# 115dkk/Impulcifer-pip313

Hardware: AMD Instinct MI355X
Metric: impulse responses/sec (sweep deconv+FIR), 7.1×2-ear @48kHz, 1/2/4/8 GPU (higher is better)
Workload: dtype f32

## Files before the change

### impulcifer-pip313_amd/csrc/conv_kernels.hip.h

```cpp
#pragma once
#include "fft_regs.hip.h"

namespace imp {

constexpr int kN2 = 4096;
constexpr int kLogN2 = 12;
constexpr int kRowPad = 272;
#ifndef IMP_AB_PREFETCH
#define IMP_AB_PREFETCH 8
#endif
constexpr int kAbPrefetch = IMP_AB_PREFETCH;

struct Twiddles {
  const cf* __restrict__ full;
  const cf* __restrict__ hi;
  const cf* __restrict__ t1;
  const cf* __restrict__ t2;
  const cf* __restrict__ t4;
};

__device__ __forceinline__ void xcd_work_item(int nchan, int& tile, int& chan) {
  const int xcd = blockIdx.x & 7;
  const int slot = blockIdx.x >> 3;
  const int tl = slot / nchan;
// ... 820 lines not shown
}

struct FirBlockArgs {
  const float4* __restrict__ ab;
  long long ab_chan_stride;
  float* __restrict__ out;
  long long out_stride;
  long long out_start, out_len;
  int kp;
  int valid;
  int blocks;
  int first_block;
  int nchan;
};

constexpr int kFirBlockPoints = 4 * kN2;
constexpr size_t kFirBlockLds = sizeof(cf) * 4 * 16 * kRowPad;

template <class L, class = void> struct LoadHasDeviceLen { static constexpr bool value = false; };
template <class L> struct LoadHasDeviceLen<L, decltype((void)L::kDeviceLen)> { static constexpr bool value = true; };

template <class Load>
__global__ __launch_bounds__(1024, 4) void fir_block_kernel(Load ld, FirBlockArgs a, Twiddles tw) {
  extern __shared__ __attribute__((aligned(16))) char smem_raw[];
  cf* lds = reinterpret_cast<cf*>(smem_raw);
  const int xcd = blockIdx.x & 7, slot = blockIdx.x >> 3;
  const int chan = (slot / a.blocks) * 8 + xcd, blk = a.first_block + slot % a.blocks;
  if (chan >= a.nchan) return;
  long long out_len = a.out_len;
  int filt = chan;
  if constexpr (LoadHasDeviceLen<Load>::value) {
    out_len = ld.out_len(chan);
    filt = ld.filter_of(chan);
    if ((long long)blk * a.valid - a.out_start >= out_len) return;
  }
  const int tid = threadIdx.x;
  const int pairq = __builtin_amdgcn_readfirstlane(tid >> 9);
  const int half = __builtin_amdgcn_readfirstlane((tid >> 8) & 1);
  const int t = tid & 255;
  const int k1 = pairq + 2 * half;
  const int s0 = blk * a.valid - a.kp;
  const __amdgpu_buffer_rsrc_t r_full = make_rsrc(tw.full, 4u * kN2 * 8u);
  const auto row = ld.open(chan);

  cf v[16];
#pragma unroll
  for (int h = 0; h < 2; ++h) {
    cf x[2][4], w[2][3];
#pragma unroll
    for (int c = 0; c < 2; ++c) {
      const int n2 = tid + 1024 * (2 * h + c);
#pragma unroll
      for (int n1 = 0; n1 < 4; ++n1) x[c][n1] = row.pair_at(s0 + 2 * (n1 * kN2 + n2));
#pragma unroll
      for (int k = 1; k < 4; ++k) w[c][k - 1] = bload_cf(r_full, (unsigned)(k * kN2 + n2) * 8u, 0u);
    }
#pragma unroll
    for (int c = 0; c < 2; ++c) {
      const int n2 = tid + 1024 * (2 * h + c);
#pragma unroll
      for (int n1 = 0; n1 < 4; ++n1) x[c][n1] = row.finish(x[c][n1], s0 + 2 * (n1 * kN2 + n2));
      bfly4<-1>(x[c][0], x[c][1], x[c][2], x[c][3]);
      lds[n2] = x[c][0];
#pragma unroll
      for (int k = 1; k < 4; ++k) lds[k * kN2 + n2] = cmul(x[c][k], w[c][k - 1]);
    }
  }
  __syncthreads();
#pragma unroll
  for (int j = 0; j < 16; ++j) v[j] = lds[k1 * kN2 + t + 256 * j];
  __syncthreads();
  const __amdgpu_buffer_rsrc_t r_ab =
      make_rsrc(a.ab + (long long)filt * a.ab_chan_stride + (long long)k1 * kN2, kN2 * sizeof(float4));
  rows_core<0, 4>(v, lds + pairq * (2 * 16 * kRowPad), half, pairq, k1, r_ab, tw, t);

  __syncthreads();
#pragma unroll
  for (int j = 0; j < 16; ++j) lds[k1 * kN2 + t + 256 * j] = v[j];
  __syncthreads();
  const __amdgpu_buffer_rsrc_t r_out = make_rsrc(a.out + (long long)chan * a.out_stride, (unsigned)out_len * 4u);
  const int o0 = blk * a.valid - a.kp - (int)a.out_start;
#pragma unroll
  for (int c = 0; c < 4; ++c) {
    const int n2 = tid + 1024 * c;
    cf w0 = lds[n2], w1 = lds[kN2 + n2], w2 = lds[2 * kN2 + n2], w3 = lds[3 * kN2 + n2];
    w1 = cmulc(w1, bload_cf(r_full, (unsigned)(kN2 + n2) * 8u, 0u));
    w2 = cmulc(w2, bload_cf(r_full, (unsigned)(2 * kN2 + n2) * 8u, 0u));
    w3 = cmulc(w3, bload_cf(r_full, (unsigned)(3 * kN2 + n2) * 8u, 0u));
    bfly4<+1>(w0, w1, w2, w3);
    const cf y[4] = {w0, w1, w2, w3};
#pragma unroll
    for (int n1 = 0; n1 < 4; ++n1) {
      const int pos = 2 * (n1 * kN2 + n2);
      if (pos < a.kp) continue;
      const unsigned off = (unsigned)(o0 + pos) * 4u;
      if (a.out_start & 1) {
        unsigned off_im = off + 4u;
        asm volatile("" : "+v"(off_im));
        __builtin_amdgcn_raw_buffer_store_b32(__float_as_uint(y[n1].x), r_out, off, 0u, 0);
        __builtin_amdgcn_raw_buffer_store_b32(__float_as_uint(y[n1].y), r_out, off_im, 0u, 0);
      } else {
        bstore_cf<kStreamAux>(y[n1], r_out, off, 0u);
      }
    }
  }
}

// ... 2 lines not shown
```

### impulcifer-pip313_amd/csrc/impulse_hip.hip

```cpp
#include <hip/hip_runtime.h>

#include <algorithm>
#include <cmath>
#include <complex>
#include <cstdarg>
#include <cstdio>
#include <cstdlib>
#include <cstring>
#include <map>
#include <mutex>
#include <new>
#include <string>
#include <vector>

#include "internal.h"
#include "conv_kernels.hip.h"
#include "ir_kernels.hip.h"
#include "decay_kernels.hip.h"
#include "slice_kernels.hip.h"

static thread_local std::string g_last_error;

int imp_fail(int code, const char* fmt, ...) {
  char buf[1024];
// ... 436 lines not shown
  int64_t nfft = 0, Nc = 0;
  bool ola = false;
  int64_t ola_lb = 0, ola_mp = 0, ola_blocks = 1, ola_parts = 1;
  int N1 = 0, R2 = 0, F = 16;
  int64_t ws_channels = 0;
  int lanes = 1;
  int64_t group_counter_lane = 0;
  hipStream_t cur_stream = nullptr;
  cf* cur_ws = nullptr;
  TwSet tw;
  float4* ab = nullptr;
  cf* ws = nullptr;
  bool fused = false;
  int f_kp = 0, f_valid = 0;
  int64_t f_first = 0, f_blocks = 0;
  bool paired = false;
  cf* hs = nullptr;
  float* d_in = nullptr;
  float* d_out = nullptr;
  size_t d_in_bytes = 0, d_out_bytes = 0;
  unsigned* tile_max = nullptr;
  int timing = 0;
  int64_t group_counter = 0;
  bool group_timed = false;
  std::vector<hipEvent_t> events;
  int64_t timed = 0;
  double acc_ms[3] = {0, 0, 0};
  int64_t acc_launches = 0;
};

// ... 104 lines not shown
  int rc_attr = ctx_kernel_lds(p->ctx, reinterpret_cast<const void*>(imp::rows_single_kernel), kRowsSingleLds);
  if (rc_attr) return rc_attr;
  imp::RowsPairArgs a;
  a.ws = p->cur_ws;
  a.hs = p->hs;
  a.n1_total = p->N1;
  a.npairs = (int)npairs;
  imp::Twiddles tw{p->tw.full, p->tw.hi, p->ctx->tw_t1, p->ctx->tw_t2, p->ctx->tw_t4};
  dim3 grid((unsigned)(npairs * ((p->N1 + 7) / 8 * 8))), block(256);
  hipLaunchKernelGGL(imp::rows_single_kernel, grid, block, kRowsSingleLds, p->cur_stream, a, tw);
  HIP_TRY(hipGetLastError());
  return IMP_OK;
}

static constexpr int64_t kFusedMaxTaps = 24577;

static int plan_geometry(imp_plan* p, int64_t M, int64_t n_filters, int64_t L, int mode, int64_t ws_channels,
                         bool paired = false, bool allow_fused = true) {
  if (M < 1 || L < 1) return fail(IMP_ERR_INVALID, "M and L must be >= 1 (M=%lld L=%lld)", (long long)M, (long long)L);
  if (n_filters < 1) return fail(IMP_ERR_INVALID, "n_filters must be >= 1");
  if (mode != IMP_MODE_SAME && mode != IMP_MODE_FULL) return fail(IMP_ERR_INVALID, "mode must be IMP_MODE_SAME or IMP_MODE_FULL");
  const int64_t full = L + M - 1;
  const int64_t need = (mode == IMP_MODE_SAME) ? std::max(L + M / 2, M) : full;
  static const struct { int f, r2; bool pair_only; } kShapes[] = {
      {4, 1, false},  {8, 1, false},  {16, 1, false}, {8, 3, false},  {16, 2, false},  {8, 5, false},
      {16, 3, false}, {16, 4, false}, {11, 6, false}, {8, 9, false},  {16, 5, false},  {16, 6, false},
      {16, 8, false}, {11, 12, true}, {16, 9, false}, {16, 10, false}, {16, 12, false}, {16, 16, false}, {16, 18, true},
      {16, 24, true}};
  const int64_t samples_per_row = paired ? imp::kN2 : 2 * imp::kN2;
  if (paired && n_filters != 1) return fail(IMP_ERR_INVALID, "pair mode needs ONE filter shared by both channels of a pair");
// ... 89 lines not shown
  if (e != hipSuccess) return fail(IMP_ERR_ALLOC, "hipMalloc(spectrum): %s", hipGetErrorString(e));
  e = hipMalloc((void**)&p->ws, p->fused ? 256 : plane * (size_t)(p->paired ? p->ws_channels / 2 : p->ws_channels) * sizeof(cf));
  if (e != hipSuccess) return fail(IMP_ERR_ALLOC, "hipMalloc(workspace): %s", hipGetErrorString(e));
  return IMP_OK;
}

static int plan_sync_lanes(imp_plan* p);

extern "C" void imp_plan_destroy(imp_plan* p) {
  if (!p) return;
  IMP_CTX_LOCK(p->ctx);
  (void)hipSetDevice(p->ctx->device);
  (void)plan_sync_lanes(p);
  if (p->ab) (void)hipFree(p->ab);
  if (p->hs) (void)hipFree(p->hs);
  if (p->ws) (void)hipFree(p->ws);
  if (p->d_in) (void)hipFree(p->d_in);
  if (p->d_out) (void)hipFree(p->d_out);
  for (auto ev : p->events) (void)hipEventDestroy(ev);
  delete p;
}

static int plan_create_empty_impl(imp_ctx* ctx, int64_t M, int64_t n_filters, int64_t L, int mode, int64_t ws_channels,
                                  bool paired, imp_plan** out, bool allow_fused = true) {
  if (!ctx || !out) return fail(IMP_ERR_INVALID, "imp_conv_plan_create_empty: null argument");
  IMP_CTX_LOCK(ctx);
  *out = nullptr;
  imp_plan* p = new (std::nothrow) imp_plan();
  if (!p) return fail(IMP_ERR_ALLOC, "out of host memory");
  p->ctx = ctx;
// ... 5 lines not shown
  }
  *out = p;
  return IMP_OK;
}

extern "C" int imp_conv_plan_create_empty(imp_ctx* ctx, int64_t M, int64_t n_filters, int64_t L, int mode,
                                          int64_t ws_channels, imp_plan** out) {
  return plan_create_empty_impl(ctx, M, n_filters, L, mode, ws_channels, false, out);
}

extern "C" int imp_conv_plan_create_empty_paired(imp_ctx* ctx, int64_t M, int64_t L, int mode, int64_t ws_channels,
                                                 imp_plan** out) {
  return plan_create_empty_impl(ctx, M, 1, L, mode, ws_channels, true, out);
}

static int plan_fill_spectrum(imp_plan* p, const double* filter, int64_t filter_ld, bool on_device = false) {
  imp_ctx* ctx = p->ctx;
  const int64_t M = p->M, n_filters = p->n_filters;
  const int64_t ld = n_filters > 1 ? filter_ld : M;
  if (on_device) {
    if (p->paired || p->ola) return fail(IMP_ERR_UNSUPPORTED, "device filters: mono and fused plans without overlap-add");
    return spectrum_alpha_beta_device(ctx, filter, M, n_filters, ld, p->Nc, p->N1, p->ab, true);
  }
  if (p->paired) return spectrum_pair_device(ctx, filter, M, p->Nc, p->N1, p->hs);
  const size_t plane = (size_t)p->N1 * imp::kN2;
  const char* host_env = std::getenv("IMPULSE_HIP_HOST_SPECTRUM");
  if (host_env && host_env[0] == '1' && !p->ola) {
    std::vector<float4> ab(plane);
    std::vector<cd> H;
    for (int64_t f = 0; f < n_filters; ++f) {
      host_rfft(filter + f * ld, M, p->Nc, H);
// ... 5 lines not shown
    }
    return IMP_OK;
  }
  if (!p->ola) return spectrum_alpha_beta_device(ctx, filter, M, n_filters, ld, p->Nc, p->N1, p->ab);
  for (int64_t j = 0; j < p->ola_parts; ++j) {
    const int64_t m0 = j * p->ola_mp, mj = std::min(p->ola_mp, M - m0);
    for (int64_t f = 0; f < n_filters; ++f) {
      int rc = spectrum_alpha_beta_device(ctx, filter + f * ld + m0, mj, 1, mj, p->Nc, p->N1,
                                          p->ab + (size_t)(f * p->ola_parts + j) * plane);
      if (rc) return rc;
    }
  }
  return IMP_OK;
}

static int plan_create_impl(imp_ctx* ctx, const double* filter, int64_t M, int64_t n_filters, int64_t filter_ld, int64_t L,
                            int mode, int64_t ws_channels, bool paired, imp_plan** out, bool allow_fused = true) {
  if (!ctx || !out) return fail(IMP_ERR_INVALID, "imp_conv_plan_create: null argument");
  if (!filter) return fail(IMP_ERR_INVALID, "imp_conv_plan_create: null filter");
  IMP_CTX_LOCK(ctx);
  if (n_filters > 1 && filter_ld < M) return fail(IMP_ERR_INVALID, "filter_ld < M");
  imp_plan* p = nullptr;
  int rc = plan_create_empty_impl(ctx, M, n_filters, L, mode, ws_channels, paired, &p, allow_fused);
  if (rc) return rc;
  if ((rc = plan_fill_spectrum(p, filter, filter_ld))) {
    imp_plan_destroy(p);
    return rc;
  }
  *out = p;
  return IMP_OK;
// ... 100 lines not shown
}

extern "C" int imp_plan_info(const imp_plan* p, int64_t* nfft, int64_t* out_len, int64_t* ws_channels,
                             int64_t* n1_rows) {
  if (!p) return fail(IMP_ERR_INVALID, "null plan");
  if (nfft) *nfft = p->nfft;
  if (out_len) *out_len = p->out_len;
  if (ws_channels) *ws_channels = p->ws_channels;
  if (n1_rows) *n1_rows = p->N1;
  return IMP_OK;
}

extern "C" int imp_plan_spectrum(imp_plan* p, void** dptr, size_t* bytes) {
  if (!p || !dptr || !bytes) return fail(IMP_ERR_INVALID, "imp_plan_spectrum: null argument");
  IMP_CTX_LOCK(p->ctx);
  if (p->paired) {
    *dptr = p->hs;
    *bytes = (size_t)p->N1 * imp::kN2 * sizeof(cf);
    return IMP_OK;
  }
  *dptr = p->ab;
  *bytes = (size_t)p->N1 * imp::kN2 * (size_t)(p->n_filters * p->ola_parts) * sizeof(float4);
  return IMP_OK;
}

extern "C" int imp_plan_copy_spectrum(imp_plan* dst, imp_plan* src) {
  if (!dst || !src) return fail(IMP_ERR_INVALID, "imp_plan_copy_spectrum: null argument");
  if (dst == src) return IMP_OK;
  if (dst->paired != src->paired || dst->fused != src->fused || dst->N1 != src->N1 || dst->M != src->M || dst->L != src->L ||
      dst->mode != src->mode || dst->n_filters != src->n_filters || dst->ola_parts != src->ola_parts)
    return fail(IMP_ERR_INVALID, "imp_plan_copy_spectrum: the two plans differ in geometry");
  void *d = nullptr, *s_ = nullptr;
  size_t nd = 0, ns = 0;
  int rc;
  if ((rc = imp_plan_spectrum(src, &s_, &ns)) || (rc = imp_plan_spectrum(dst, &d, &nd))) return rc;
  if (nd != ns) return fail(IMP_ERR_INVALID, "imp_plan_copy_spectrum: spectrum sizes differ");
  {
    IMP_CTX_LOCK(src->ctx);
    if ((rc = ctx_bind(src->ctx))) return rc;
    HIP_TRY(hipStreamSynchronize(src->ctx->stream));
  }
  IMP_CTX_LOCK(dst->ctx);
  if ((rc = ctx_bind(dst->ctx))) return rc;
  if ((rc = plan_sync_lanes(dst))) return rc;
  HIP_TRY(hipMemcpyPeerAsync(d, dst->ctx->device, s_, src->ctx->device, ns, dst->ctx->stream));
  HIP_TRY(hipStreamSynchronize(dst->ctx->stream));
  return IMP_OK;
}

extern "C" int imp_memcpy_peer(imp_ctx* dst_ctx, void* dst, imp_ctx* src_ctx, const void* src, size_t bytes) {
// ... 70 lines not shown
  const size_t need = (size_t)(4 * (p->timed + 1));
  while (p->events.size() < need) {
    hipEvent_t ev;
    HIP_TRY(hipEventCreate(&ev));
    p->events.push_back(ev);
  }
  HIP_TRY(hipEventRecord(p->events[(size_t)(4 * p->timed + slot)], p->cur_stream));
  if (slot == 3) ++p->timed;
  return IMP_OK;
}

template <class Load>
static int run_group_with(imp_plan* p, Load ld, int64_t nchan, float* d_y, int64_t chan_stride_out,
                          int64_t first_chan, int last_stage);

template <class Load>
static int launch_fir_block(imp_plan* p, Load ld, int64_t nchan, float* d_y, int64_t chan_stride_out, int64_t first_chan) {
  auto kern = imp::fir_block_kernel<Load>;
  int rc = ctx_kernel_lds(p->ctx, reinterpret_cast<const void*>(kern), imp::kFirBlockLds);
  if (rc) return rc;
  const int64_t plane = (int64_t)4 * imp::kN2;
  imp::FirBlockArgs a;
  a.ab = p->ab + (p->n_filters > 1 ? first_chan * plane : 0);
  a.ab_chan_stride = p->n_filters > 1 ? plane : 0;
  a.out = d_y;
  a.out_stride = chan_stride_out;
  a.out_start = p->out_start;
  a.first_block = (int)p->f_first;
  a.out_len = p->out_len;
  a.kp = p->f_kp;
  a.valid = p->f_valid;
  a.blocks = (int)p->f_blocks;
  a.nchan = (int)nchan;
  imp::Twiddles tw{p->tw.full, p->tw.hi, p->ctx->tw_t1, p->ctx->tw_t2, p->ctx->tw_t4};
  dim3 grid((unsigned)((nchan + 7) / 8 * 8 * p->f_blocks)), block(1024);
  hipLaunchKernelGGL(kern, grid, block, imp::kFirBlockLds, p->cur_stream, ld, a, tw);
  HIP_TRY(hipGetLastError());
  return IMP_OK;
}

template <class Load>
static int run_group_pair(imp_plan* p, Load ld, int64_t nchan, float* d_y, int64_t chan_stride_out, int last_stage) {
  int rc;
  const int64_t lane_channels = p->ws_channels / p->lanes;
  const int lane = (p->lanes > 1) ? (int)(p->group_counter_lane++ % p->lanes) : 0;
  p->cur_stream = lane ? p->ctx->side_streams[(size_t)(lane - 1)] : p->ctx->stream;
  p->cur_ws = p->ws + (int64_t)lane * (lane_channels / 2) * p->N1 * imp::kN2;
  if (nchan < 1 || nchan > lane_channels || (lane_channels & 1))
    return fail(IMP_ERR_INVALID, "launch group of %lld channels exceeds the workspace lane (%lld, whole pairs)",
                (long long)nchan, (long long)lane_channels);
  const int64_t npairs = (nchan + 1) / 2;
  if ((double)(chan_stride_out + p->out_len) * 4.0 >= 4294967296.0)
    return fail(IMP_ERR_INVALID, "chan_stride_out %lld: a pair's two output rows must lie within 4 GiB", (long long)chan_stride_out);
// ... 388 lines not shown
  int64_t B = 0, n = 0, head = 0, fade_in = 0, fade_out = 0, pitch_ir = 0;
  double peak_height = 0.12589;
  int lanes = 1;
  int sets = 1;
  int64_t calls = 0;
  int tiles = 0;
  int64_t chunks = 0;
  std::vector<float*> d_ir;
  std::vector<unsigned*> d_tile;
  std::vector<imp::RowPeak*> d_res;
  std::vector<hipEvent_t> k1_done;
  std::vector<hipEvent_t> ir_free;
  std::vector<char> ir_busy;
  int64_t* d_meta = nullptr;
  double* d_win = nullptr;
};

struct ChainLock {
  std::unique_lock<std::recursive_mutex> a, b;
  ChainLock(imp_ctx* x, imp_ctx* y) {
    if (x == y) {
      a = std::unique_lock<std::recursive_mutex>(x->mu);
    } else {
      imp_ctx* lo = x < y ? x : y;
      imp_ctx* hi = x < y ? y : x;
      a = std::unique_lock<std::recursive_mutex>(lo->mu);
      b = std::unique_lock<std::recursive_mutex>(hi->mu);
    }
  }
};

extern "C" void imp_chain_destroy(imp_chain* c) {
  if (!c) return;
  ChainLock lk(c->ctx, c->tail_ctx);
  (void)hipSetDevice(c->ctx->device);
  (void)plan_sync_lanes(c->deconv);
  (void)hipStreamSynchronize(c->tail_ctx->stream);
  for (auto p : c->d_ir) (void)hipFree(p);
  for (auto p : c->d_tile) (void)hipFree(p);
  for (auto p : c->d_res) (void)hipFree(p);
  for (auto e : c->k1_done) (void)hipEventDestroy(e);
  for (auto e : c->ir_free) (void)hipEventDestroy(e);
  (void)hipFree(c->d_meta);
  (void)hipFree(c->d_win);
  delete c;
}

extern "C" int imp_chain_create(imp_plan* deconv, imp_plan* fir, int64_t B, int64_t head, int64_t fade_in, int64_t fade_out,
                                double peak_height, imp_chain** out) {
  if (!deconv || !fir || !out) return fail(IMP_ERR_INVALID, "imp_chain_create: null argument");
  *out = nullptr;
  if (deconv->ctx->device != fir->ctx->device) return fail(IMP_ERR_INVALID, "imp_chain_create: the two plans live on different devices");
  ChainLock lk(deconv->ctx, fir->ctx);
  if (deconv->mode != IMP_MODE_SAME || fir->mode != IMP_MODE_FULL)
    return fail(IMP_ERR_INVALID, "imp_chain_create: needs a 'same' deconvolution plan and a 'full' FIR plan");
  if (!(peak_height > 0.0)) return fail(IMP_ERR_INVALID, "imp_chain_create: peak_height must be positive (got %g)", peak_height);
  if (fir->lanes != 1) return fail(IMP_ERR_INVALID, "imp_chain_create: the FIR plan must run in stream order (lanes = 1)");
  if (deconv->lanes > 1 && deconv->ctx == fir->ctx)
    return fail(IMP_ERR_INVALID, "imp_chain_create: a deconvolution plan with several lanes needs the FIR plan on a context of its own "
// ... 48 lines not shown
    unsigned* tile = nullptr;
    imp::RowPeak* res = nullptr;
    hipEvent_t e1 = nullptr, e2 = nullptr;
    ok = hipMalloc((void**)&ir, (size_t)(B * c->pitch_ir) * sizeof(float)) == hipSuccess;
    if (ir) c->d_ir.push_back(ir);
    ok = ok && hipMalloc((void**)&tile, chunk_bytes * (size_t)c->tiles) == hipSuccess;
    if (tile) c->d_tile.push_back(tile);
    ok = ok && hipMalloc((void**)&res, (size_t)B * sizeof(imp::RowPeak)) == hipSuccess;
    if (res) c->d_res.push_back(res);
    ok = ok && hipEventCreateWithFlags(&e1, hipEventDisableTiming) == hipSuccess;
    if (e1) c->k1_done.push_back(e1);
    ok = ok && hipEventCreateWithFlags(&e2, hipEventDisableTiming) == hipSuccess;
    if (e2) c->ir_free.push_back(e2);
  }
  c->ir_busy.assign((size_t)c->sets, 0);
  if (!ok) {
    (void)hipGetLastError();
    imp_chain_destroy(c);
    return fail(IMP_ERR_ALLOC, "imp_chain_create: device allocation failed");
  }
  *out = c;
  return IMP_OK;
}

extern "C" int imp_chain_execute_device(imp_chain* c, const float* d_x, int64_t chan_stride_in, int64_t elem_stride_in,
                                        float* d_out, int64_t chan_stride_out, long long* d_peaks_out) {
  if (!c || !d_x || !d_out) return fail(IMP_ERR_INVALID, "imp_chain_execute_device: null argument");
  ChainLock lk(c->ctx, c->tail_ctx);
  if (chan_stride_out < c->fir->out_len)
    return fail(IMP_ERR_INVALID, "chan_stride_out %lld < out_len %lld", (long long)chan_stride_out, (long long)c->fir->out_len);
// ... 9 lines not shown
  c->deconv->tile_max = c->d_tile[(size_t)l];
  rc = imp_conv_execute_device(c->deconv, d_x, c->B, chan_stride_in, elem_stride_in, c->d_ir[(size_t)l], c->pitch_ir);
  c->deconv->tile_max = nullptr;
  if (rc) return rc;
  if (c->deconv->cur_stream != lane_stream) return fail(IMP_ERR_HIP, "imp_chain_execute_device: lane bookkeeping out of step");
  if (tail != lane_stream) {
    HIP_TRY(hipEventRecord(c->k1_done[(size_t)l], lane_stream));
    HIP_TRY(hipStreamWaitEvent(tail, c->k1_done[(size_t)l], 0));
  }
  hipLaunchKernelGGL(imp::row_first_peak_chunked_kernel, dim3((unsigned)c->B), dim3(imp::kPeakThreads), 0, tail, c->d_ir[(size_t)l],
                     c->d_meta, c->d_meta + c->B, c->deconv->out_start, (const unsigned*)c->d_tile[(size_t)l], c->tiles,
                     (const unsigned*)nullptr, c->chunks, c->d_res[(size_t)l], c->peak_height, d_peaks_out);
  HIP_TRY(hipGetLastError());
  imp::LoadCropAtPeak ld{c->d_ir[(size_t)l], c->pitch_ir, c->deconv->out_len, c->d_res[(size_t)l], c->n, c->head, c->fade_in, c->fade_out,
                         c->d_win};
  if ((rc = run_group_with(c->fir, ld, c->B, d_out, chan_stride_out, 0, 2))) return rc;
  if (tail != lane_stream) {
    HIP_TRY(hipEventRecord(c->ir_free[(size_t)l], tail));
    c->ir_busy[(size_t)l] = 1;
  }
  return IMP_OK;
}

struct imp_segset {
  imp_ctx* ctx = nullptr;
  int64_t B = 0;
  double* e = nullptr;
  int64_t* off = nullptr;
  int64_t* len = nullptr;
  std::vector<int64_t> h_len;
  void* qbuf = nullptr;
  size_t qcap = 0;
  void* keep_a = nullptr;
  void* keep_b = nullptr;
  std::vector<int64_t> keep_host;
// ... 671 lines not shown
```

### impulcifer-pip313_amd/impulse_hip/_native.py

```python
import atexit
import ctypes as C
import os
import threading
import weakref

import numpy as np

_HERE = os.path.dirname(os.path.abspath(__file__))
_DEFAULT_LIB = os.path.normpath(os.path.join(_HERE, "..", "csrc", "libimpulse_hip.so"))

IMP_MODE_SAME = 0
IMP_MODE_FULL = 1
IMP_ERR_UNSUPPORTED = -3


class NativeUnavailable(RuntimeError):
    """libimpulse_hip.so is missing or no MI355X (gfx950) device is usable."""


class NativeError(RuntimeError):

    def __init__(self, code, message):
        super().__init__(f"impulse_hip error {code}: {message}")
        self.code = code
# ... 75 lines not shown
    "imp_plan_kind": (C.c_int, [_vp, C.POINTER(C.c_int)]),
    "imp_conv_execute_device_pairs": (C.c_int, [_vp, _vp, C.c_int, _i64, _i64, _i64, _i64, _vp, _i64]),
    "imp_plan_destroy": (None, [_vp]),
    "imp_plan_info": (C.c_int, [_vp, _pi64, _pi64, _pi64, _pi64]),
    "imp_plan_spectrum": (C.c_int, [_vp, C.POINTER(_vp), C.POINTER(C.c_size_t)]),
    "imp_plan_copy_spectrum": (C.c_int, [_vp, _vp]),
    "imp_memcpy_peer": (C.c_int, [_vp, _vp, _vp, _vp, C.c_size_t]),
    "imp_conv_execute": (C.c_int, [_vp, _pf, _i64, _i64, _pf, _i64]),
    "imp_conv_execute_interleaved": (C.c_int, [_vp, _pf, _i64, _pf, _i64]),
    "imp_conv_execute_device": (C.c_int, [_vp, _vp, _i64, _i64, _i64, _vp, _i64]),
    "imp_conv_execute_device_pcm": (C.c_int, [_vp, _vp, C.c_int, _i64, _i64, _i64, _vp, _i64]),
    "imp_plan_set_overlap": (C.c_int, [_vp, C.c_int]),
    "imp_chain_create": (C.c_int, [_vp, _vp, _i64, _i64, _i64, _i64, C.c_double, C.POINTER(_vp)]),
    "imp_chain_execute_device": (C.c_int, [_vp, _vp, _i64, _i64, _vp, _i64, _vp]),
    "imp_chain_destroy": (None, [_vp]),
    "imp_slice_create": (C.c_int, [_vp, C.POINTER(SliceGeometry), _i64, C.POINTER(_vp)]),
    "imp_slice_destroy": (None, [_vp]),
    "imp_slice_info": (C.c_int, [_vp, _pi64, _pi64, _pi64, _pi64]),
    "imp_slice_set_firs": (C.c_int, [_vp, _pd, _i64]),
    "imp_slice_execute_device": (C.c_int, [_vp, _vp, _i64, _i64, _vp, _i64]),
    "imp_slice_results": (C.c_int, [_vp, C.POINTER(SliceRowResult), C.POINTER(SliceResult)]),
    "imp_slice_set_decay": (C.c_int, [_vp, _pd]),
    "imp_slice_set_alignment": (C.c_int, [_vp, _i64, C.POINTER(C.c_int32), C.POINTER(C.c_int32), C.POINTER(C.c_int32), C.c_int32, _i64]),
    "imp_xcorr_argmax_device": (C.c_int, [_vp, _vp, _pi64, _pi64, _pi64, _pi64, _i64, _pi64, _pd]),
    "imp_shift_rows_device": (C.c_int, [_vp, _vp, _pi64, _pi64, _pi64, _i64, _vp, _pi64]),
    "imp_slice_pack_f64": (C.c_int, [_vp, _vp, _i64, _i64, _vp, _i64]),
    "imp_host_alloc": (C.c_int, [_vp, C.c_size_t, C.POINTER(_vp)]),
    "imp_host_free": (C.c_int, [_vp]),
    "imp_comm_unique_id": (C.c_int, [C.POINTER(C.c_ubyte)]),
    "imp_comm_create": (C.c_int, [_vp, C.POINTER(C.c_ubyte), C.c_int, C.c_int, C.POINTER(_vp)]),
    "imp_comm_destroy": (None, [_vp]),
    "imp_comm_probe": (C.c_int, []),
    "imp_comm_nranks": (C.c_int, [_vp, C.POINTER(C.c_int)]),
    "imp_comm_broadcast": (C.c_int, [_vp, _vp, C.c_size_t, C.c_int]),
    "imp_plan_broadcast_spectrum": (C.c_int, [_vp, _vp, C.c_int, C.POINTER(C.c_size_t)]),
    "imp_plan_set_filters": (C.c_int, [_vp, _pd, _i64]),
    "imp_plan_set_filters_device": (C.c_int, [_vp, _vp, _i64]),
    "imp_curves_equalization_fir_device": (C.c_int, [_vp, _pd, _i64, C.c_int, C.c_double, C.c_double, C.c_double, C.c_double,
                                                     C.c_double, C.c_int, C.c_double, C.c_double, C.c_int, _pd, C.POINTER(_vp), _pi64]),
    "imp_slice_set_firs_device": (C.c_int, [_vp, _vp, _i64]),
    "imp_plan_set_timing": (C.c_int, [_vp, C.c_int]),
    "imp_plan_get_timing": (C.c_int, [_vp, _pd, _pi64, C.c_int]),
    "imp_debug_plan_geometry": (C.c_int, [_i64, _i64, C.c_int, _pi64, _pi64, _pi64]),
    "imp_debug_plan_geometry_fused": (C.c_int, [_i64, _i64, C.c_int, _pi64, _pi64, _pi64, _pi64]),
    "imp_debug_plan_geometry_paired": (C.c_int, [_i64, _i64, C.c_int, _pi64, _pi64, _pi64, _pi64]),
    "imp_debug_host_spectrum": (C.c_int, [_pd, _i64, C.c_int, _pf]),
    "imp_plan_debug_run_stage": (C.c_int, [_vp, _pf, _i64, _i64, C.c_int, _pf]),
    "imp_segset_create": (C.c_int, [_vp, _pd, _pi64, _pi64, _i64, C.POINTER(_vp), _pd]),
    "imp_segset_range_means": (C.c_int, [_vp, _pi64, _pi64, _pi64, _i64, _pd]),
    "imp_segset_destroy": (None, [_vp]),
    "imp_decay_times": (C.c_int, [_vp, _pd, _pi64, _pi64, _i64, _pi64, _pi64, _pd, _pi64, C.c_double, _pd]),
    "imp_decay_times_device": (C.c_int, [_vp, _vp, _pi64, _pi64, _i64, _pi64, _pi64, _pd, _pi64, C.c_double, _pd]),
    "imp_sosfilt": (C.c_int, [_vp, _pd, _i64, _pd, _pi64, _pi64, _i64, _pd]),
    "imp_xcorr_argmax": (C.c_int, [_vp, _pd, _pi64, _pi64, _pd, _pi64, _pi64, _i64, _pi64, _pd]),
    "imp_minphase_fir": (C.c_int, [_vp, _pd, _i64, _i64, C.c_double, _pd]),
    "imp_curves_create": (C.c_int, [_vp, _pd, _i64, C.POINTER(_vp)]),
    "imp_curves_destroy": (None, [_vp]),
    "imp_curves_window_size": (C.c_int, [_vp, C.c_double, C.POINTER(C.c_int)]),
    "imp_curves_smooth": (C.c_int, [_vp, _pd, _i64, C.c_double, C.c_double, C.c_double, C.c_double, _pd]),
# ... 453 lines not shown
        self.ctx = deconv_plan.ctx
        self._lib = self.ctx._lib
        self._plans = (deconv_plan, fir_plan)
        h = _vp()
        _check(self._lib.imp_chain_create(deconv_plan.handle, fir_plan.handle, int(B), int(head), int(fade_in),
                                          int(fade_out), float(peak_height), C.byref(h)))
        self._h = h
        self.ctx._plans.add(self)
        fir_plan.ctx._plans.add(self)

    def execute_device(self, d_x, chan_stride_in, d_out, chan_stride_out, d_peaks=0, elem_stride_in=1):
        if not getattr(self, "_h", None):
            raise NativeError(-1, "the chain is closed (one of its contexts was closed)")
        _check(self._lib.imp_chain_execute_device(self._h, _vp(int(d_x)), int(chan_stride_in), int(elem_stride_in),
                                                  _vp(int(d_out)), int(chan_stride_out), _vp(int(d_peaks)) if d_peaks else None))

    def close(self):
        if getattr(self, "_h", None):
            if all(getattr(p.ctx, "_h", None) for p in self._plans):
                self._lib.imp_chain_destroy(self._h)
            self._h = None

    def __del__(self):
        try:
            self.close()
        except Exception:
            pass


class Slice:
# ... 557 lines not shown
                                       C.byref(a), C.byref(b), C.byref(c)))
    return a.value, b.value, c.value


def plan_geometry_fused(M, L, mode="same"):
    lib = load_library()
    a, b, c, d = _i64(), _i64(), _i64(), _i64()
    rc = lib.imp_debug_plan_geometry_fused(int(M), int(L), {"same": IMP_MODE_SAME, "full": IMP_MODE_FULL}[mode],
                                           C.byref(a), C.byref(b), C.byref(c), C.byref(d))
    if rc == IMP_ERR_UNSUPPORTED:
        return None
    _check(rc)
    return a.value, b.value, c.value, d.value


def plan_geometry_paired(M, L, mode="same"):
    lib = load_library()
    a, b, c, d = _i64(), _i64(), _i64(), _i64()
    rc = lib.imp_debug_plan_geometry_paired(int(M), int(L), {"same": IMP_MODE_SAME, "full": IMP_MODE_FULL}[mode],
                                            C.byref(a), C.byref(b), C.byref(c), C.byref(d))
    if rc == IMP_ERR_UNSUPPORTED:
        return None
    _check(rc)
    return a.value, b.value, c.value, d.value


def host_spectrum(filt, n1_rows):
    lib = load_library()
    f = np.ascontiguousarray(filt, dtype=np.float64)
    out = np.empty((int(n1_rows), 4096, 4), dtype=np.float32)
# ... 77 lines not shown
```

### include/impulse_hip.h

```cpp
#ifndef IMPULSE_HIP_H_
#define IMPULSE_HIP_H_

#include <stdint.h>
#include <stddef.h>

#ifdef __cplusplus
extern "C" {
#endif

#define IMP_OK 0
#define IMP_ERR_INVALID (-1)
#define IMP_ERR_HIP (-2)
#define IMP_ERR_UNSUPPORTED (-3)
#define IMP_ERR_NO_DEVICE (-4)
#define IMP_ERR_ALLOC (-5)

#define IMP_MODE_SAME 0
#define IMP_MODE_FULL 1

typedef struct imp_ctx imp_ctx;
typedef struct imp_plan imp_plan;

const char* imp_version(void);
const char* imp_last_error(void);
// ... 150 lines not shown
                           int64_t* window_out, int32_t* flags_out);
int imp_rows_to_pcm_device(imp_ctx* ctx, const float* d_rows, const int64_t* off, const int64_t* len, int64_t n_rows,
                           const int64_t* row_of_track, int64_t n_tracks, int64_t n_frames, int bits, void* pcm_out);
int imp_magnitude_db_sum_device(imp_ctx* ctx, const float* d_rows, const int64_t* off, const int64_t* len,
                                const int64_t* group, int64_t n_rows, int64_t n_groups, int64_t n, double* db_out);
int imp_magnitude_db_sum_peak_device(imp_ctx* ctx, const float* d_rows, const int64_t* off, const int64_t* len,
                                     const int64_t* group, int64_t n_rows, int64_t n_groups, int64_t n,
                                     double* peak_db_out);

typedef struct imp_chain imp_chain;
int imp_chain_create(imp_plan* deconv, imp_plan* fir, int64_t B, int64_t head, int64_t fade_in, int64_t fade_out,
                     double peak_height, imp_chain** out);
int imp_chain_execute_device(imp_chain* chain, const float* d_x, int64_t chan_stride_in, int64_t elem_stride_in,
                             float* d_out, int64_t chan_stride_out, long long* d_peaks_out);
void imp_chain_destroy(imp_chain* chain);

#define IMP_SLICE_KNEE_GUARD 1
#define IMP_SLICE_KNEE_RANGE 2
#define IMP_SLICE_KEEP_CAP 4
#define IMP_SLICE_FADE 8
#define IMP_SLICE_GAIN_GUARD 16
#define IMP_SLICE_GAIN_NONFINITE 32
#define IMP_SLICE_SHORT 64
#define IMP_SLICE_ALIGN_GUARD 256
#define IMP_SLICE_DECAY_GUARD 128
typedef struct imp_slice imp_slice;
typedef struct imp_slice_geometry {
  int64_t n_pairs;
  int64_t elem_stride;
  int bits;
// ... 66 lines not shown
```

Baseline: 300,700.

## Add 2-row fused FIR block kernel for chain tail with short filters

Templates the fused FIR block kernel on the number of rows (2 or 4). The chain's FIR stage uses a 512-thread, 8192-point block variant when the filter has at most 12289 taps. The tail needs a separate alpha/beta spectrum at the smaller size, so the plan now keeps device copies of the filter taps, uses generation counters to track staleness, and rebuilds the spectrum lazily. The smaller FFT is meant to cut wasted transform work on short filters, at the cost of more blocks and an extra spectrum buffer per chain.

```diff
diff --git a/impulcifer-pip313_amd/csrc/conv_kernels.hip.h b/impulcifer-pip313_amd/csrc/conv_kernels.hip.h
--- a/impulcifer-pip313_amd/csrc/conv_kernels.hip.h
+++ b/impulcifer-pip313_amd/csrc/conv_kernels.hip.h
@@ -858,14 +858,29 @@
   int nchan;
 };
 
-constexpr int kFirBlockPoints = 4 * kN2;
-constexpr size_t kFirBlockLds = sizeof(cf) * 4 * 16 * kRowPad;
+template <int N1>
+struct FirBlockCfg {
+  static_assert(N1 == 2 || N1 == 4, "fir_block_kernel holds two or four rows");
+  static constexpr int kThreads = 256 * N1;
+  static constexpr int kPoints = N1 * kN2;
+  static constexpr size_t kLds = sizeof(cf) * N1 * 16 * kRowPad;
+  static constexpr int kAbPrefetch = N1 == 4 ? 4 : ::imp::kAbPrefetch;
+};
+constexpr int kFirBlockPoints = FirBlockCfg<4>::kPoints;
+constexpr size_t kFirBlockLds = FirBlockCfg<4>::kLds;
 
 template <class L, class = void> struct LoadHasDeviceLen { static constexpr bool value = false; };
 template <class L> struct LoadHasDeviceLen<L, decltype((void)L::kDeviceLen)> { static constexpr bool value = true; };
 
-template <class Load>
-__global__ __launch_bounds__(1024, 4) void fir_block_kernel(Load ld, FirBlockArgs a, Twiddles tw) {
+template <int N1>
+__device__ __forceinline__ cf fir_twiddle(__amdgpu_buffer_rsrc_t r_full, int k1, int n2) {
+  return bload_cf(r_full, (unsigned)((k1 * (4 / N1)) * kN2 + n2) * 8u, 0u);
+}
+
+template <int N1, class Load>
+__global__ __launch_bounds__(FirBlockCfg<N1>::kThreads, 4) void fir_block_kernel(Load ld, FirBlockArgs a, Twiddles tw) {
+  using Cfg = FirBlockCfg<N1>;
+  constexpr int T = Cfg::kThreads;
   extern __shared__ __attribute__((aligned(16))) char smem_raw[];
   cf* lds = reinterpret_cast<cf*>(smem_raw);
   const int xcd = blockIdx.x & 7, slot = blockIdx.x >> 3;
@@ -879,35 +894,38 @@
     if ((long long)blk * a.valid - a.out_start >= out_len) return;
   }
   const int tid = threadIdx.x;
-  const int pairq = __builtin_amdgcn_readfirstlane(tid >> 9);
+  const int pairq = N1 == 4 ? __builtin_amdgcn_readfirstlane(tid >> 9) : 0;
   const int half = __builtin_amdgcn_readfirstlane((tid >> 8) & 1);
   const int t = tid & 255;
-  const int k1 = pairq + 2 * half;
+  const int k1 = pairq + (N1 / 2) * half;
   const int s0 = blk * a.valid - a.kp;
   const __amdgpu_buffer_rsrc_t r_full = make_rsrc(tw.full, 4u * kN2 * 8u);
   const auto row = ld.open(chan);
 
+  constexpr int CPT = kN2 / T;
+  constexpr int CH = 8 / N1;
   cf v[16];
 #pragma unroll
-  for (int h = 0; h < 2; ++h) {
-    cf x[2][4], w[2][3];
-#pragma unroll
-    for (int c = 0; c < 2; ++c) {
-      const int n2 = tid + 1024 * (2 * h + c);
-#pragma unroll
-      for (int n1 = 0; n1 < 4; ++n1) x[c][n1] = row.pair_at(s0 + 2 * (n1 * kN2 + n2));
-#pragma unroll
-      for (int k = 1; k < 4; ++k) w[c][k - 1] = bload_cf(r_full, (unsigned)(k * kN2 + n2) * 8u, 0u);
-    }
-#pragma unroll
-    for (int c = 0; c < 2; ++c) {
-      const int n2 = tid + 1024 * (2 * h + c);
-#pragma unroll
-      for (int n1 = 0; n1 < 4; ++n1) x[c][n1] = row.finish(x[c][n1], s0 + 2 * (n1 * kN2 + n2));
-      bfly4<-1>(x[c][0], x[c][1], x[c][2], x[c][3]);
+  for (int h = 0; h < CPT / CH; ++h) {
+    cf x[CH][N1], w[CH][N1 - 1];
+#pragma unroll
+    for (int c = 0; c < CH; ++c) {
+      const int n2 = tid + T * (CH * h + c);
+#pragma unroll
+      for (int n1 = 0; n1 < N1; ++n1) x[c][n1] = row.pair_at(s0 + 2 * (n1 * kN2 + n2));
+#pragma unroll
+      for (int k = 1; k < N1; ++k) w[c][k - 1] = fir_twiddle<N1>(r_full, k, n2);
+    }
+#pragma unroll
+    for (int c = 0; c < CH; ++c) {
+      const int n2 = tid + T * (CH * h + c);
+#pragma unroll
+      for (int n1 = 0; n1 < N1; ++n1) x[c][n1] = row.finish(x[c][n1], s0 + 2 * (n1 * kN2 + n2));
+      if constexpr (N1 == 4) bfly4<-1>(x[c][0], x[c][1], x[c][2], x[c][3]);
+      else bfly2<-1>(x[c][0], x[c][1]);
       lds[n2] = x[c][0];
 #pragma unroll
-      for (int k = 1; k < 4; ++k) lds[k * kN2 + n2] = cmul(x[c][k], w[c][k - 1]);
+      for (int k = 1; k < N1; ++k) lds[k * kN2 + n2] = cmul(x[c][k], w[c][k - 1]);
     }
   }
   __syncthreads();
@@ -916,7 +934,7 @@
   __syncthreads();
   const __amdgpu_buffer_rsrc_t r_ab =
       make_rsrc(a.ab + (long long)filt * a.ab_chan_stride + (long long)k1 * kN2, kN2 * sizeof(float4));
-  rows_core<0, 4>(v, lds + pairq * (2 * 16 * kRowPad), half, pairq, k1, r_ab, tw, t);
+  rows_core<0, Cfg::kAbPrefetch>(v, lds + pairq * (2 * 16 * kRowPad), half, pairq, k1, r_ab, tw, t);
 
   __syncthreads();
 #pragma unroll
@@ -925,16 +943,17 @@
   const __amdgpu_buffer_rsrc_t r_out = make_rsrc(a.out + (long long)chan * a.out_stride, (unsigned)out_len * 4u);
   const int o0 = blk * a.valid - a.kp - (int)a.out_start;
 #pragma unroll
-  for (int c = 0; c < 4; ++c) {
-    const int n2 = tid + 1024 * c;
-    cf w0 = lds[n2], w1 = lds[kN2 + n2], w2 = lds[2 * kN2 + n2], w3 = lds[3 * kN2 + n2];
-    w1 = cmulc(w1, bload_cf(r_full, (unsigned)(kN2 + n2) * 8u, 0u));
-    w2 = cmulc(w2, bload_cf(r_full, (unsigned)(2 * kN2 + n2) * 8u, 0u));
-    w3 = cmulc(w3, bload_cf(r_full, (unsigned)(3 * kN2 + n2) * 8u, 0u));
-    bfly4<+1>(w0, w1, w2, w3);
-    const cf y[4] = {w0, w1, w2, w3};
-#pragma unroll
-    for (int n1 = 0; n1 < 4; ++n1) {
+  for (int c = 0; c < CPT; ++c) {
+    const int n2 = tid + T * c;
+    cf y[N1];
+#pragma unroll
+    for (int k = 0; k < N1; ++k) y[k] = lds[k * kN2 + n2];
+#pragma unroll
+    for (int k = 1; k < N1; ++k) y[k] = cmulc(y[k], fir_twiddle<N1>(r_full, k, n2));
+    if constexpr (N1 == 4) bfly4<+1>(y[0], y[1], y[2], y[3]);
+    else bfly2<+1>(y[0], y[1]);
+#pragma unroll
+    for (int n1 = 0; n1 < N1; ++n1) {
       const int pos = 2 * (n1 * kN2 + n2);
       if (pos < a.kp) continue;
       const unsigned off = (unsigned)(o0 + pos) * 4u;
diff --git a/impulcifer-pip313_amd/csrc/impulse_hip.hip b/impulcifer-pip313_amd/csrc/impulse_hip.hip
--- a/impulcifer-pip313_amd/csrc/impulse_hip.hip
+++ b/impulcifer-pip313_amd/csrc/impulse_hip.hip
@@ -474,6 +474,8 @@
   bool fused = false;
   int f_kp = 0, f_valid = 0;
   int64_t f_first = 0, f_blocks = 0;
+  int64_t filter_gen = 0, taps_gen = -1;
+  double* d_taps = nullptr;
   bool paired = false;
   cf* hs = nullptr;
   float* d_in = nullptr;
@@ -608,6 +610,7 @@
 }
 
 static constexpr int64_t kFusedMaxTaps = 24577;
+static constexpr int64_t kChainTail2MaxTaps = 16384 - 4096 + 1;
 
 static int plan_geometry(imp_plan* p, int64_t M, int64_t n_filters, int64_t L, int mode, int64_t ws_channels,
                          bool paired = false, bool allow_fused = true) {
@@ -727,6 +730,7 @@
   (void)plan_sync_lanes(p);
   if (p->ab) (void)hipFree(p->ab);
   if (p->hs) (void)hipFree(p->hs);
+  if (p->d_taps) (void)hipFree(p->d_taps);
   if (p->ws) (void)hipFree(p->ws);
   if (p->d_in) (void)hipFree(p->d_in);
   if (p->d_out) (void)hipFree(p->d_out);
@@ -762,7 +766,7 @@
   return plan_create_empty_impl(ctx, M, 1, L, mode, ws_channels, true, out);
 }
 
-static int plan_fill_spectrum(imp_plan* p, const double* filter, int64_t filter_ld, bool on_device = false) {
+static int plan_fill_planes(imp_plan* p, const double* filter, int64_t filter_ld, bool on_device) {
   imp_ctx* ctx = p->ctx;
   const int64_t M = p->M, n_filters = p->n_filters;
   const int64_t ld = n_filters > 1 ? filter_ld : M;
@@ -798,6 +802,24 @@
   return IMP_OK;
 }
 
+static int plan_fill_spectrum(imp_plan* p, const double* filter, int64_t filter_ld, bool on_device = false) {
+  ++p->filter_gen;
+  int rc = plan_fill_planes(p, filter, filter_ld, on_device);
+  if (rc || !p->fused || p->M > kChainTail2MaxTaps) return rc;
+  const int64_t ld = p->n_filters > 1 ? filter_ld : p->M;
+  const size_t row = (size_t)p->M * sizeof(double);
+  if (!p->d_taps && hipMalloc((void**)&p->d_taps, row * (size_t)p->n_filters) != hipSuccess) {
+    (void)hipGetLastError();
+    p->d_taps = nullptr;
+    return IMP_OK;
+  }
+  HIP_TRY(hipMemcpy2DAsync(p->d_taps, row, filter, (size_t)ld * sizeof(double), row, (size_t)p->n_filters,
+                           on_device ? hipMemcpyDeviceToDevice : hipMemcpyHostToDevice, p->ctx->stream));
+  if (!on_device) HIP_TRY(hipStreamSynchronize(p->ctx->stream));
+  p->taps_gen = p->filter_gen;
+  return IMP_OK;
+}
+
 static int plan_create_impl(imp_ctx* ctx, const double* filter, int64_t M, int64_t n_filters, int64_t filter_ld, int64_t L,
                             int mode, int64_t ws_channels, bool paired, imp_plan** out, bool allow_fused = true) {
   if (!ctx || !out) return fail(IMP_ERR_INVALID, "imp_conv_plan_create: null argument");
@@ -928,6 +950,7 @@
 extern "C" int imp_plan_spectrum(imp_plan* p, void** dptr, size_t* bytes) {
   if (!p || !dptr || !bytes) return fail(IMP_ERR_INVALID, "imp_plan_spectrum: null argument");
   IMP_CTX_LOCK(p->ctx);
+  ++p->filter_gen;
   if (p->paired) {
     *dptr = p->hs;
     *bytes = (size_t)p->N1 * imp::kN2 * sizeof(cf);
@@ -947,7 +970,9 @@
   void *d = nullptr, *s_ = nullptr;
   size_t nd = 0, ns = 0;
   int rc;
+  const int64_t src_gen = src->filter_gen;
   if ((rc = imp_plan_spectrum(src, &s_, &ns)) || (rc = imp_plan_spectrum(dst, &d, &nd))) return rc;
+  src->filter_gen = src_gen;
   if (nd != ns) return fail(IMP_ERR_INVALID, "imp_plan_copy_spectrum: spectrum sizes differ");
   {
     IMP_CTX_LOCK(src->ctx);
@@ -1048,29 +1073,36 @@
 static int run_group_with(imp_plan* p, Load ld, int64_t nchan, float* d_y, int64_t chan_stride_out,
                           int64_t first_chan, int last_stage);
 
-template <class Load>
-static int launch_fir_block(imp_plan* p, Load ld, int64_t nchan, float* d_y, int64_t chan_stride_out, int64_t first_chan) {
-  auto kern = imp::fir_block_kernel<Load>;
-  int rc = ctx_kernel_lds(p->ctx, reinterpret_cast<const void*>(kern), imp::kFirBlockLds);
-  if (rc) return rc;
-  const int64_t plane = (int64_t)4 * imp::kN2;
+template <int N1, class Load>
+static int launch_fir_block_rows(imp_plan* p, Load ld, int64_t nchan, float* d_y, int64_t chan_stride_out, const float4* ab,
+                                 int kp, int valid, int64_t first, int64_t blocks) {
+  using Cfg = imp::FirBlockCfg<N1>;
+  auto kern = imp::fir_block_kernel<N1, Load>;
+  int rc = ctx_kernel_lds(p->ctx, reinterpret_cast<const void*>(kern), Cfg::kLds);
+  if (rc) return rc;
   imp::FirBlockArgs a;
-  a.ab = p->ab + (p->n_filters > 1 ? first_chan * plane : 0);
-  a.ab_chan_stride = p->n_filters > 1 ? plane : 0;
+  a.ab = ab;
+  a.ab_chan_stride = p->n_filters > 1 ? (int64_t)N1 * imp::kN2 : 0;
   a.out = d_y;
   a.out_stride = chan_stride_out;
   a.out_start = p->out_start;
-  a.first_block = (int)p->f_first;
+  a.first_block = (int)first;
   a.out_len = p->out_len;
-  a.kp = p->f_kp;
-  a.valid = p->f_valid;
-  a.blocks = (int)p->f_blocks;
+  a.kp = kp;
+  a.valid = valid;
+  a.blocks = (int)blocks;
   a.nchan = (int)nchan;
   imp::Twiddles tw{p->tw.full, p->tw.hi, p->ctx->tw_t1, p->ctx->tw_t2, p->ctx->tw_t4};
-  dim3 grid((unsigned)((nchan + 7) / 8 * 8 * p->f_blocks)), block(1024);
-  hipLaunchKernelGGL(kern, grid, block, imp::kFirBlockLds, p->cur_stream, ld, a, tw);
+  dim3 grid((unsigned)((nchan + 7) / 8 * 8 * blocks)), block(Cfg::kThreads);
+  hipLaunchKernelGGL(kern, grid, block, Cfg::kLds, p->cur_stream, ld, a, tw);
   HIP_TRY(hipGetLastError());
   return IMP_OK;
+}
+
+template <class Load>
+static int launch_fir_block(imp_plan* p, Load ld, int64_t nchan, float* d_y, int64_t chan_stride_out, int64_t first_chan) {
+  const float4* ab = p->ab + (p->n_filters > 1 ? first_chan * (int64_t)imp::kFirBlockPoints : 0);
+  return launch_fir_block_rows<4>(p, ld, nchan, d_y, chan_stride_out, ab, p->f_kp, p->f_valid, p->f_first, p->f_blocks);
 }
 
 template <class Load>
@@ -1489,7 +1521,37 @@
   std::vector<char> ir_busy;
   int64_t* d_meta = nullptr;
   double* d_win = nullptr;
+  float4* d_ab2 = nullptr;
+  int64_t ab2_gen = -1;
+  int t2_kp = 0, t2_valid = 0;
+  int64_t t2_first = 0, t2_blocks = 0;
 };
+
+static bool chain_tail2_geometry(int64_t M, int64_t out_start, int64_t out_len, int* kp, int* valid, int64_t* first,
+                                 int64_t* blocks) {
+  if (M < 1 || M > kChainTail2MaxTaps) return false;
+  *kp = (int)((M - 1 + 1) & ~(int64_t)1);
+  *valid = (int)(2 * imp::FirBlockCfg<2>::kPoints - *kp);
+  *first = out_start / *valid;
+  *blocks = (out_start + out_len - 1) / *valid - *first + 1;
+  return true;
+}
+
+static int chain_tail2_prepare(imp_chain* c, bool* ready) {
+  imp_plan* f = c->fir;
+  *ready = false;
+  if (!c->d_ab2) return IMP_OK;
+  if (c->ab2_gen == f->filter_gen) {
+    *ready = true;
+    return IMP_OK;
+  }
+  if (!f->d_taps || f->taps_gen != f->filter_gen) return IMP_OK;
+  int rc = spectrum_alpha_beta_device(f->ctx, f->d_taps, f->M, f->n_filters, f->M, imp::FirBlockCfg<2>::kPoints, 2, c->d_ab2, true);
+  if (rc) return rc;
+  c->ab2_gen = f->filter_gen;
+  *ready = true;
+  return IMP_OK;
+}
 
 struct ChainLock {
   std::unique_lock<std::recursive_mutex> a, b;
@@ -1518,6 +1580,7 @@
   for (auto e : c->ir_free) (void)hipEventDestroy(e);
   (void)hipFree(c->d_meta);
   (void)hipFree(c->d_win);
+  (void)hipFree(c->d_ab2);
   delete c;
 }
 
@@ -1596,6 +1659,17 @@
     if (e2) c->ir_free.push_back(e2);
   }
   c->ir_busy.assign((size_t)c->sets, 0);
+  const char* k5_env = std::getenv("IMPULSE_HIP_CHAIN_K5");
+  const bool block4 = k5_env && std::strcmp(k5_env, "block4") == 0;
+  if (ok && fir->fused && !block4 &&
+      chain_tail2_geometry(fir->M, fir->out_start, fir->out_len, &c->t2_kp, &c->t2_valid, &c->t2_first, &c->t2_blocks)) {
+    ok = hipMalloc((void**)&c->d_ab2, (size_t)fir->n_filters * imp::FirBlockCfg<2>::kPoints * sizeof(float4)) == hipSuccess;
+    bool ready = false;
+    if (ok && (rc = chain_tail2_prepare(c, &ready))) {
+      imp_chain_destroy(c);
+      return rc;
+    }
+  }
   if (!ok) {
     (void)hipGetLastError();
     imp_chain_destroy(c);
@@ -1635,11 +1709,45 @@
   HIP_TRY(hipGetLastError());
   imp::LoadCropAtPeak ld{c->d_ir[(size_t)l], c->pitch_ir, c->deconv->out_len, c->d_res[(size_t)l], c->n, c->head, c->fade_in, c->fade_out,
                          c->d_win};
-  if ((rc = run_group_with(c->fir, ld, c->B, d_out, chan_stride_out, 0, 2))) return rc;
+  bool tail2 = false;
+  if ((rc = chain_tail2_prepare(c, &tail2))) return rc;
+  if (tail2) {
+    imp_plan* f = c->fir;
+    f->cur_stream = f->ctx->stream;
+    if ((rc = timing_event(f, 0))) return rc;
+    if ((rc = launch_fir_block_rows<2>(f, ld, c->B, d_out, chan_stride_out, c->d_ab2, c->t2_kp, c->t2_valid, c->t2_first,
+                                       c->t2_blocks)))
+      return rc;
+    for (int slot = 1; slot <= 3; ++slot)
+      if ((rc = timing_event(f, slot))) return rc;
+  } else if ((rc = run_group_with(c->fir, ld, c->B, d_out, chan_stride_out, 0, 2))) {
+    return rc;
+  }
   if (tail != lane_stream) {
     HIP_TRY(hipEventRecord(c->ir_free[(size_t)l], tail));
     c->ir_busy[(size_t)l] = 1;
   }
+  return IMP_OK;
+}
+
+extern "C" int imp_chain_tail_rows(imp_chain* c, int* rows) {
+  if (!c || !rows) return fail(IMP_ERR_INVALID, "imp_chain_tail_rows: null argument");
+  ChainLock lk(c->ctx, c->tail_ctx);
+  imp_plan* f = c->fir;
+  *rows = c->d_ab2 && (c->ab2_gen == f->filter_gen || (f->d_taps && f->taps_gen == f->filter_gen)) ? 2 : 4;
+  return IMP_OK;
+}
+
+extern "C" int imp_debug_chain_tail_geometry(int64_t M, int64_t L, int64_t* history, int64_t* valid, int64_t* blocks) {
+  if (L < 1) return fail(IMP_ERR_INVALID, "L must be >= 1 (got %lld)", (long long)L);
+  int kp = 0, v = 0;
+  int64_t first = 0, nb = 0;
+  if (!chain_tail2_geometry(M, 0, L + M - 1, &kp, &v, &first, &nb))
+    return fail(IMP_ERR_UNSUPPORTED, "the chain's 2-row K5 takes 1 to %lld taps (got %lld)", (long long)kChainTail2MaxTaps,
+                (long long)M);
+  if (history) *history = kp;
+  if (valid) *valid = v;
+  if (blocks) *blocks = nb;
   return IMP_OK;
 }
 
diff --git a/impulcifer-pip313_amd/impulse_hip/_native.py b/impulcifer-pip313_amd/impulse_hip/_native.py
--- a/impulcifer-pip313_amd/impulse_hip/_native.py
+++ b/impulcifer-pip313_amd/impulse_hip/_native.py
@@ -113,6 +113,7 @@
     "imp_chain_create": (C.c_int, [_vp, _vp, _i64, _i64, _i64, _i64, C.c_double, C.POINTER(_vp)]),
     "imp_chain_execute_device": (C.c_int, [_vp, _vp, _i64, _i64, _vp, _i64, _vp]),
     "imp_chain_destroy": (None, [_vp]),
+    "imp_chain_tail_rows": (C.c_int, [_vp, C.POINTER(C.c_int)]),
     "imp_slice_create": (C.c_int, [_vp, C.POINTER(SliceGeometry), _i64, C.POINTER(_vp)]),
     "imp_slice_destroy": (None, [_vp]),
     "imp_slice_info": (C.c_int, [_vp, _pi64, _pi64, _pi64, _pi64]),
@@ -142,6 +143,7 @@
     "imp_plan_get_timing": (C.c_int, [_vp, _pd, _pi64, C.c_int]),
     "imp_debug_plan_geometry": (C.c_int, [_i64, _i64, C.c_int, _pi64, _pi64, _pi64]),
     "imp_debug_plan_geometry_fused": (C.c_int, [_i64, _i64, C.c_int, _pi64, _pi64, _pi64, _pi64]),
+    "imp_debug_chain_tail_geometry": (C.c_int, [_i64, _i64, _pi64, _pi64, _pi64]),
     "imp_debug_plan_geometry_paired": (C.c_int, [_i64, _i64, C.c_int, _pi64, _pi64, _pi64, _pi64]),
     "imp_debug_host_spectrum": (C.c_int, [_pd, _i64, C.c_int, _pf]),
     "imp_plan_debug_run_stage": (C.c_int, [_vp, _pf, _i64, _i64, C.c_int, _pf]),
@@ -625,6 +627,11 @@
             raise NativeError(-1, "the chain is closed (one of its contexts was closed)")
         _check(self._lib.imp_chain_execute_device(self._h, _vp(int(d_x)), int(chan_stride_in), int(elem_stride_in),
                                                   _vp(int(d_out)), int(chan_stride_out), _vp(int(d_peaks)) if d_peaks else None))
+
+    def tail_rows(self):
+        r = C.c_int()
+        _check(self._lib.imp_chain_tail_rows(self._h, C.byref(r)))
+        return r.value
 
     def close(self):
         if getattr(self, "_h", None):
@@ -1212,6 +1219,16 @@
     return a.value, b.value, c.value, d.value
 
 
+def chain_tail_geometry(M, L):
+    lib = load_library()
+    a, b, c = _i64(), _i64(), _i64()
+    rc = lib.imp_debug_chain_tail_geometry(int(M), int(L), C.byref(a), C.byref(b), C.byref(c))
+    if rc == IMP_ERR_UNSUPPORTED:
+        return None
+    _check(rc)
+    return a.value, b.value, c.value
+
+
 def plan_geometry_paired(M, L, mode="same"):
     lib = load_library()
     a, b, c, d = _i64(), _i64(), _i64(), _i64()
diff --git a/include/impulse_hip.h b/include/impulse_hip.h
--- a/include/impulse_hip.h
+++ b/include/impulse_hip.h
@@ -188,6 +188,8 @@
 int imp_chain_execute_device(imp_chain* chain, const float* d_x, int64_t chan_stride_in, int64_t elem_stride_in,
                              float* d_out, int64_t chan_stride_out, long long* d_peaks_out);
 void imp_chain_destroy(imp_chain* chain);
+int imp_chain_tail_rows(imp_chain* chain, int* rows);
+int imp_debug_chain_tail_geometry(int64_t M, int64_t L, int64_t* history, int64_t* valid, int64_t* blocks);
 
 #define IMP_SLICE_KNEE_GUARD 1
 #define IMP_SLICE_KNEE_RANGE 2
```

Result: faster. 314,100, median of 6 (+4.5%).
